# efirdc/Segmentation-Pipeline

Hardware: AMD Instinct MI355X
Metric: 3D patches/sec (128³, 4ch) train+infer at 1/2/4/8 MI355X; Dice vs CPU ref (higher is better)
Workload: dtype f32 (tensors, results and accumulation; the products of the 3x3x3 convolutions with >= 8 input channels run as six bf16 MFMAs on an EXACT three-way bf16 split of both f32 operands -- error vs f64 equal to the f32 MFMA kernels', profiles/r04_f32x3_accuracy.txt; the same step on v_mfma_f32_32x32x2_f32

## Files before the change

### include/m355seg.h

```cpp
#ifndef M355SEG_H
#define M355SEG_H

#include <stddef.h>
#include <stdint.h>

#ifdef __cplusplus
extern "C" {
#endif

#define M355_ABI_VERSION 3

enum {
  M355_OK = 0,
  M355_EINVALID_ARG = -1,
  M355_EUNSUPPORTED = -2,
  M355_ELAUNCH = -3,
  M355_EWORKSPACE = -4
};

enum { M355_F32 = 0 };

enum { M355_COMPUTE_F32 = 0, M355_COMPUTE_BF16 = 1, M355_COMPUTE_F16 = 2, M355_COMPUTE_F32X3 = 3 };

enum { M355_ACT_NONE = 0, M355_ACT_RELU = 1, M355_ACT_LEAKY_RELU = 2, M355_ACT_ELU = 3, M355_ACT_GELU = 4,
// ... 81 lines not shown
size_t m355_conv_transpose3d_workspace(const m355_conv3d_desc* d);
int m355_conv_transpose3d_fwd(const m355_conv3d_desc* d, const float* x, const float* w,
                              const float* bias, float* y,
                              void* workspace, size_t workspace_bytes, void* stream);
int m355_conv_transpose3d_bwd_data(const m355_conv3d_desc* d, const float* dy, const float* w,
                                   float* dx, void* workspace, size_t workspace_bytes,
                                   void* stream);
int m355_conv_transpose3d_bwd_weight(const m355_conv3d_desc* d, const float* x, const float* dy,
                                     float* dw, float* dbias,
                                     void* workspace, size_t workspace_bytes, void* stream);

int m355_conv_transpose3d_plan(const m355_conv3d_desc* d, int32_t which, const void* y_side, int32_t* out4);

int m355_conv_transpose3d_fwd_h16(const m355_conv3d_desc* d, const void* x16, int64_t x16_batch_stride,
                                  const float* w, const float* bias, void* y16, int64_t y16_batch_stride,
                                  int32_t compute, void* stream);

typedef struct m355_norm_desc {
  int32_t N, C;
  int64_t S;
  int32_t groups;
  int32_t act;
  float eps;
  float act_slope;
  int64_t x_batch_stride;
  int64_t y_batch_stride;
  int64_t add_batch_stride;
} m355_norm_desc;

int64_t m355_norm_num_stats(const m355_norm_desc* d);
size_t m355_norm_workspace(const m355_norm_desc* d);

int m355_norm_plan(const m355_norm_desc* d, int32_t which, int32_t* out4);

int m355_norm_stats(const m355_norm_desc* d, const float* x, float* mean, float* rstd,
                    float* running_mean, float* running_var, float momentum,
                    void* workspace, size_t workspace_bytes, void* stream);
int m355_norm_stats_from_partials(const m355_norm_desc* d, const float* stat_partials, int64_t slots,
                                  float* mean, float* rstd, float* running_mean, float* running_var,
                                  float momentum, void* workspace, size_t workspace_bytes, void* stream);
int m355_norm_stats_from_running(const m355_norm_desc* d, const float* running_mean,
                                 const float* running_var, float* mean, float* rstd,
                                 void* stream);
int m355_norm_act_fwd(const m355_norm_desc* d, const float* x, const float* mean,
                      const float* rstd, const float* gamma, const float* beta,
                      const float* add, float* y, void* stream);
int m355_norm_act_pool_fwd(const m355_norm_desc* d, const float* x, const float* mean, const float* rstd,
                           const float* gamma, const float* beta, float* y, float* pooled, int64_t pooled_batch_stride,
                           int32_t D, int32_t H, int32_t W, void* stream);
int m355_norm_act_bwd(const m355_norm_desc* d, const float* x, const float* dy,
                      const float* mean, const float* rstd, const float* gamma,
                      const float* beta, float* dx, float* dgamma, float* dbeta,
                      int training, void* workspace, size_t workspace_bytes, void* stream);
int m355_norm_act_bwd_h16(const m355_norm_desc* d, const float* x, const float* dy, const float* mean,
                          const float* rstd, const float* gamma, const float* beta, float* dx, float* dgamma,
                          float* dbeta, int training, void* dx16, int64_t dx16_batch_stride, int32_t compute,
                          void* workspace, size_t workspace_bytes, void* stream);

int m355_norm_sums(const m355_norm_desc* d, const float* x, const float* stat_partials, int64_t slots, double* sums,
                   void* workspace, size_t workspace_bytes, void* stream);
int m355_norm_stats_from_sums(const m355_norm_desc* d, const double* sums, float* mean, float* rstd,
                              float* running_mean, float* running_var, float momentum, void* stream);
int m355_norm_act_bwd_reduce(const m355_norm_desc* d, const float* x, const float* dy, const float* mean,
                             const float* rstd, const float* gamma, const float* beta, float* dgamma, float* dbeta,
                             int training, const double* total_count, float* stat_m, void* workspace,
                             size_t workspace_bytes, void* stream);
int m355_norm_act_bwd_apply(const m355_norm_desc* d, const float* x, const float* dy, const float* mean,
                            const float* rstd, const float* gamma, const float* beta, const float* stat_m, float* dx,
                            void* dx16, int64_t dx16_batch_stride, int32_t compute, void* stream);

int m355_norm_act_fwd_h16(const m355_norm_desc* d, const float* x, const float* mean, const float* rstd,
                          const float* gamma, const float* beta, const float* add, float* y, void* y16,
                          int64_t y16_batch_stride, int32_t compute, void* stream);
int m355_norm_act_fwd_c8(const m355_norm_desc* d, const void* x16, int64_t x16_batch_stride, const float* mean,
                         const float* rstd, const float* gamma, const float* beta, const void* add16,
                         int64_t add16_batch_stride, void* y16, int64_t y16_batch_stride, int32_t compute,
                         void* stream);
int64_t m355_act16_partials_slots(int64_t S);
int m355_act16_channel_partials(const void* x16, int64_t x16_batch_stride, int32_t N, int32_t C, int64_t S,
                                int32_t compute, float* stat_partials, void* stream);
int m355_avgpool3d_2x_fwd_h16(const void* x16, void* y16, int32_t N, int32_t C, int32_t D, int32_t H, int32_t W,
                              int64_t x16_batch_stride, int64_t y16_batch_stride, int32_t compute, void* stream);

int m355_act16_pack_scaled(const float* x, void* x16, int32_t N, int32_t C, int64_t S, int64_t x_batch_stride,
                           int64_t x16_batch_stride, int32_t compute, float scale, void* stream);
int m355_act16_unpack_scaled(const void* x16, float* x, int32_t N, int32_t C, int64_t S, int64_t x16_batch_stride,
                             int64_t x_batch_stride, int32_t compute, float scale, void* stream);
int m355_conv3d_bwd_data_h16_c8(const m355_conv3d_desc* d, const void* dy16, int64_t dy16_batch_stride, const float* w,
                                void* dx16, int64_t dx16_batch_stride, void* workspace, size_t workspace_bytes,
                                void* stream);
size_t m355_conv3d_bwd_weight_c8_workspace(const m355_conv3d_desc* d);
int m355_conv3d_bwd_weight_c8(const m355_conv3d_desc* d, const void* x16, int64_t x16_batch_stride, const void* dy16,
                              int64_t dy16_batch_stride, float* dw, float* dbias, float grad_unscale, void* workspace,
                              size_t workspace_bytes, void* stream);
int m355_norm_act_bwd_c8(const m355_norm_desc* d, const void* x16, int64_t x16_batch_stride, const void* dy16,
                         int64_t dy16_batch_stride, const void* dpool16, int64_t dpool16_batch_stride, int32_t D,
                         int32_t H, int32_t W, const float* mean, const float* rstd, const float* gamma,
                         const float* beta, void* dx16, int64_t dx16_batch_stride, float* dgamma, float* dbeta,
                         int training, float grad_unscale, int32_t compute, void* workspace, size_t workspace_bytes,
                         void* stream);
int m355_norm_act_bwd_c8_reduce(const m355_norm_desc* d, const void* x16, int64_t x16_batch_stride, const void* dy16,
                                int64_t dy16_batch_stride, const void* dpool16, int64_t dpool16_batch_stride, int32_t D,
                                int32_t H, int32_t W, const float* mean, const float* rstd, const float* gamma,
                                const float* beta, float* dgamma, float* dbeta, int training, const double* total_count,
                                float grad_unscale, float* stat_m, int32_t compute, void* workspace, size_t workspace_bytes,
                                void* stream);
// ... 338 lines not shown
```

### segmentation-pipeline_amd/_lib.py

```python
import ctypes as C
import os

_HERE = os.path.dirname(os.path.abspath(__file__))
LIB_PATH = os.environ.get("M355_LIB_PATH") or os.path.join(_HERE, "libm355seg.so")

M355_OK = 0
ACT_NONE, ACT_RELU, ACT_LEAKY_RELU = 0, 1, 2
ACT_ELU, ACT_GELU, ACT_GELU_TANH, ACT_SILU = 3, 4, 5, 6
COMPUTE_F32, COMPUTE_BF16, COMPUTE_F16, COMPUTE_F32X3 = 0, 1, 2, 3
CONV_W_PACKED, CONV_SOFTMAX, CONV_SIGMOID = 1, 2, 4


class ConvDesc(C.Structure):
    _fields_ = [
        ("N", C.c_int32), ("Cin", C.c_int32), ("Cout", C.c_int32),
        ("D", C.c_int32), ("H", C.c_int32), ("W", C.c_int32),
        ("k", C.c_int32), ("stride", C.c_int32), ("pad", C.c_int32), ("out_pad", C.c_int32),
        ("x_batch_stride", C.c_int64), ("y_batch_stride", C.c_int64),
        ("compute", C.c_int32), ("flags", C.c_int32),
    ]


class PackItem(C.Structure):
    _fields_ = [("desc", ConvDesc), ("which", C.c_int32), ("w", C.c_void_p), ("packed", C.c_void_p)]
# ... 112 lines not shown
    "m355_conv3d_fwd_h16": (C.c_int, [_CD, _P, _i64, _P, _P, _P, _P, _P, _P, _sz, _P]),
    "m355_conv3d_stats_slots_c8": (_i64, [_CD]),
    "m355_conv3d_fwd_h16_c8": (C.c_int, [_CD, _P, _i64, _P, _P, _P, _i64, _P, _P, _sz, _P]),
    "m355_conv3d_bwd_data_h16": (C.c_int, [_CD, _P, _i64, _P, _P, _P, _sz, _P]),
    "m355_conv3d_bwd_weight_h16_workspace": (_sz, [_CD]),
    "m355_conv3d_bwd_weight_h16": (C.c_int, [_CD, _P, _i64, _P, _i64, _P, _P, _P, _P, _sz, _P]),
    "m355_norm_act_fwd_h16": (C.c_int, [_ND, _P, _P, _P, _P, _P, _P, _P, _P, _i64, _i32, _P]),
    "m355_norm_act_fwd_c8": (C.c_int, [_ND, _P, _i64, _P, _P, _P, _P, _P, _i64, _P, _i64, _i32, _P]),
    "m355_act16_partials_slots": (_i64, [_i64]),
    "m355_act16_channel_partials": (C.c_int, [_P, _i64, _i32, _i32, _i64, _i32, _P, _P]),
    "m355_avgpool3d_2x_fwd_h16": (C.c_int, [_P, _P, _i32, _i32, _i32, _i32, _i32, _i64, _i64, _i32, _P]),
    "m355_act16_pack_scaled": (C.c_int, [_P, _P, _i32, _i32, _i64, _i64, _i64, _i32, _f32, _P]),
    "m355_act16_unpack_scaled": (C.c_int, [_P, _P, _i32, _i32, _i64, _i64, _i64, _i32, _f32, _P]),
    "m355_conv3d_bwd_data_h16_c8": (C.c_int, [_CD, _P, _i64, _P, _P, _i64, _P, _sz, _P]),
    "m355_conv3d_bwd_weight_c8_workspace": (_sz, [_CD]),
    "m355_conv3d_bwd_weight_c8": (C.c_int, [_CD, _P, _i64, _P, _i64, _P, _P, _f32, _P, _sz, _P]),
    "m355_norm_act_bwd_c8": (C.c_int, [_ND, _P, _i64, _P, _i64, _P, _i64, _i32, _i32, _i32, _P, _P, _P, _P, _P, _i64, _P, _P,
                                       C.c_int, _f32, _i32, _P, _sz, _P]),
    "m355_norm_act_bwd_c8_reduce": (C.c_int, [_ND, _P, _i64, _P, _i64, _P, _i64, _i32, _i32, _i32, _P, _P, _P, _P, _P, _P,
                                              C.c_int, _P, _f32, _P, _i32, _P, _sz, _P]),
    "m355_norm_act_bwd_c8_apply": (C.c_int, [_ND, _P, _i64, _P, _i64, _P, _i64, _i32, _i32, _i32, _P, _P, _P, _P, _P, _P, _i64,
                                             _i32, _P]),
    "m355_avgpool3d_2x_bwd_h16": (C.c_int, [_P, _P, _P, _i32, _i32, _i32, _i32, _i32, _i64, _i64, _i64, _i32, _P]),
    "m355_upsample_trilinear2x_fwd_h16": (C.c_int, [_P, _P, _i32, _i32, _i32, _i32, _i32, _i64, _i64, _i32, _P]),
    "m355_upsample_trilinear2x_bwd_h16": (C.c_int, [_P, _P, _i32, _i32, _i32, _i32, _i32, _i64, _i64, _i32, _P]),
    "m355_act16_channel_scale": (C.c_int, [_P, _P, _P, _i32, _i32, _i64, _i64, _i64, _i32, _P]),
    "m355_space_to_depth2_h16": (C.c_int, [_P, _P, _i32, _i32, _i32, _i32, _i32, _i64, _i64, _i32, _P]),
    "m355_depth_to_space2_h16": (C.c_int, [_P, _P, _i32, _i32, _i32, _i32, _i32, _i64, _i64, _i32, _P]),
    "m355_conv_transpose3d_h16_bwd_supported": (_i32, [_CD]),
    "m355_conv_transpose3d_h16_bwd_workspace": (_sz, [_CD]),
    "m355_conv_transpose3d_bwd_data_h16": (C.c_int, [_CD, _P, _i64, _P, _P, _i64, _i32, _P]),
    "m355_conv_transpose3d_bwd_weight_h16": (C.c_int, [_CD, _P, _i64, _P, _i64, _P, _P, _f32, _i32, _P, _sz, _P]),
    "m355_conv3d_plan": (C.c_int, [_CD, _i32, C.POINTER(C.c_int32)]),
    "m355_conv3d_launch_plan": (C.c_int, [_i32, _CD, C.POINTER(_i64), C.POINTER(C.c_uint64), _sz, C.POINTER(_i64)]),
    "m355_conv3d_bwd_data_workspace": (_sz, [_CD]),
    "m355_conv3d_bwd_data": (C.c_int, [_CD, _P, _P, _P, _P, _sz, _P]),
    "m355_conv3d_bwd_weight_workspace": (_sz, [_CD]),
    "m355_conv3d_bwd_weight": (C.c_int, [_CD, _P, _P, _P, _P, _P, _sz, _P]),
    "m355_conv_transpose3d_workspace": (_sz, [_CD]),
    "m355_conv_transpose3d_plan": (C.c_int, [_CD, _i32, _P, C.POINTER(C.c_int32)]),
    "m355_conv_transpose3d_fwd": (C.c_int, [_CD, _P, _P, _P, _P, _P, _sz, _P]),
    "m355_conv_transpose3d_bwd_data": (C.c_int, [_CD, _P, _P, _P, _P, _sz, _P]),
    "m355_conv_transpose3d_bwd_weight": (C.c_int, [_CD, _P, _P, _P, _P, _P, _sz, _P]),
    "m355_conv_transpose3d_fwd_h16": (C.c_int, [_CD, _P, _i64, _P, _P, _P, _i64, _i32, _P]),
    "m355_norm_num_stats": (_i64, [_ND]),
    "m355_norm_workspace": (_sz, [_ND]),
    "m355_norm_plan": (C.c_int, [_ND, _i32, C.POINTER(C.c_int32)]),
    "m355_norm_stats": (C.c_int, [_ND, _P, _P, _P, _P, _P, _f32, _P, _sz, _P]),
    "m355_norm_stats_from_partials": (C.c_int, [_ND, _P, _i64, _P, _P, _P, _P, _f32, _P, _sz, _P]),
    "m355_norm_stats_from_running": (C.c_int, [_ND, _P, _P, _P, _P, _P]),
    "m355_norm_act_fwd": (C.c_int, [_ND, _P, _P, _P, _P, _P, _P, _P, _P]),
    "m355_norm_act_pool_fwd": (C.c_int, [_ND, _P, _P, _P, _P, _P, _P, _P, _i64, _i32, _i32, _i32, _P]),
    "m355_norm_act_bwd": (C.c_int, [_ND, _P, _P, _P, _P, _P, _P, _P, _P, _P, C.c_int, _P, _sz, _P]),
    "m355_norm_sums": (C.c_int, [_ND, _P, _P, _i64, _P, _P, _sz, _P]),
    "m355_norm_stats_from_sums": (C.c_int, [_ND, _P, _P, _P, _P, _P, _f32, _P]),
    "m355_norm_act_bwd_reduce": (C.c_int, [_ND, _P, _P, _P, _P, _P, _P, _P, _P, C.c_int, _P, _P, _P, _sz, _P]),
    "m355_norm_act_bwd_apply": (C.c_int, [_ND, _P, _P, _P, _P, _P, _P, _P, _P, _P, _i64, _i32, _P]),
    "m355_norm_act_bwd_h16": (C.c_int, [_ND, _P, _P, _P, _P, _P, _P, _P, _P, _P, C.c_int, _P, _i64, _i32, _P, _sz, _P]),
    "m355_resample_plan": (C.c_int, [_i32, _i32, _i32, _i32, _i32, _i32, C.POINTER(_i64), C.POINTER(C.c_uint64), _i32,
                                     C.POINTER(_i64)]),
    "m355_avgpool3d_2x_fwd": (C.c_int, [_P, _P, _i32, _i32, _i32, _i32, _i32, _i64, _i64, _P]),
    "m355_avgpool3d_2x_bwd": (C.c_int, [_P, _P, _i32, _i32, _i32, _i32, _i32, _i64, _i64, _P]),
    "m355_avgpool3d_2x_bwd_add": (C.c_int, [_P, _P, _P, _i32, _i32, _i32, _i32, _i32, _i64, _i64, _i64, _P]),
    "m355_maxpool3d_2x_fwd": (C.c_int, [_P, _P, _P, _i32, _i32, _i32, _i32, _i32, _i64, _i64, _P]),
    "m355_maxpool3d_2x_bwd": (C.c_int, [_P, _P, _P, _P, _i32, _i32, _i32, _i32, _i32, _i64, _i64, _i64, _P]),
    "m355_maxpool3d_2x_fwd_h16": (C.c_int, [_P, _P, _P, _i32, _i32, _i32, _i32, _i32, _i64, _i64, _i32, _P]),
    "m355_maxpool3d_2x_bwd_h16": (C.c_int, [_P, _P, _P, _P, _i32, _i32, _i32, _i32, _i32, _i64, _i64, _i64, _i32, _P]),
    "m355_upsample_trilinear2x_fwd": (C.c_int, [_P, _P, _i32, _i32, _i32, _i32, _i32, _i64, _i64, _P]),
    "m355_upsample_trilinear2x_bwd": (C.c_int, [_P, _P, _i32, _i32, _i32, _i32, _i32, _i64, _i64, _P]),
    "m355_upsample_nearest2x_fwd": (C.c_int, [_P, _P, _i32, _i32, _i32, _i32, _i32, _i64, _i64, _P]),
    "m355_upsample_nearest2x_bwd": (C.c_int, [_P, _P, _i32, _i32, _i32, _i32, _i32, _i64, _i64, _P]),
    "m355_upsample_trilinear2x_hp_fwd": (C.c_int, [_P, _P, _i32, _i32, _i32, _i32, _i32, _i64, _i64, _P]),
    "m355_upsample_trilinear2x_hp_bwd": (C.c_int, [_P, _P, _i32, _i32, _i32, _i32, _i32, _i64, _i64, _P]),
    "m355_upsample_nearest2x_fwd_h16": (C.c_int, [_P, _P, _i32, _i32, _i32, _i32, _i32, _i64, _i64, _i32, _P]),
    "m355_upsample_nearest2x_bwd_h16": (C.c_int, [_P, _P, _i32, _i32, _i32, _i32, _i32, _i64, _i64, _i32, _P]),
    "m355_upsample_trilinear2x_hp_fwd_h16": (C.c_int, [_P, _P, _i32, _i32, _i32, _i32, _i32, _i64, _i64, _i32, _P]),
    "m355_upsample_trilinear2x_hp_bwd_h16": (C.c_int, [_P, _P, _i32, _i32, _i32, _i32, _i32, _i64, _i64, _i32, _P]),
    "m355_upsample2x_plan": (C.c_int, [_i32, _i32, _i32, _i32, _i32, _i32, _i32, _i32, C.POINTER(_i64), C.POINTER(C.c_uint64),
                                       _i32, C.POINTER(_i64)]),
    "m355_softmax_fwd": (C.c_int, [_P, _P, _i32, _i32, _i32, _i64, _f32, _P]),
    "m355_softmax_bwd": (C.c_int, [_P, _P, _P, _i32, _i32, _i32, _i64, _P]),
    "m355_sigmoid_fwd": (C.c_int, [_P, _P, _i64, _P]),
    "m355_sigmoid_bwd": (C.c_int, [_P, _P, _P, _i64, _P]),
    "m355_hybrid_loss_workspace": (_sz, [_i32, _i32, _i64]),
    "m355_hybrid_loss_fwd": (C.c_int, [_P, _P, _i32, _i32, _i64, _f32, _P, _i32, _P, _P, _P, _sz, _P]),
    "m355_hybrid_loss_bwd": (C.c_int, [_P, _P, _P, _P, _i32, _i32, _i64, _f32, _P, _i32, _P, _P]),
    "m355_binary_loss_workspace": (_sz, [_i32, _i32, _i64]),
    "m355_binary_loss_fwd": (C.c_int, [_P, _P, _i32, _i32, _i64, _f32, _P, _P, _i32, _i32, _P, _P, _P, _sz, _P]),
    "m355_binary_loss_bwd": (C.c_int, [_P, _P, _P, _P, _i32, _i32, _i64, _f32, _P, _P, _i32, _i32, _P, _P]),
    "m355_copy_channels": (C.c_int, [_P, _P, _i32, _i32, _i64, _i64, _i64, _P]),
    "m355_channel_scale": (C.c_int, [_P, _P, _P, _i32, _i32, _i64, _P]),
    "m355_add": (C.c_int, [_P, _P, _P, _i64, _P]),
    "m355_space_to_depth2": (C.c_int, [_P, _P, _i32, _i32, _i32, _i32, _i32, _i64, _i64, _P]),
    "m355_depth_to_space2": (C.c_int, [_P, _P, _i32, _i32, _i32, _i32, _i32, _i64, _i64, _P]),
    "m355_blur_weight_fwd": (C.c_int, [_P, _P, _P, _P, _i32, _i32, _i32, _i32, _P]),
    "m355_blur_weight_bwd": (C.c_int, [_P, _P, _P, _P, _P, _i32, _i32, _i32, _i32, _P]),
    "m355_weight_standardize_fwd": (C.c_int, [_P, _P, _P, _i32, _i32, _P]),
    "m355_weight_standardize_bwd": (C.c_int, [_P, _P, _P, _P, _i32, _i32, _P]),
    "m355_sampler_table_bytes": (_sz, [_i32, _i32, _i32]),
    "m355_sampler_build": (C.c_int, [_P] + [_i32] * 6 + [_P, _P]),
    "m355_sampler_draw": (C.c_int, [_P, _P] + [_i32] * 6 + [_P, _i32, _P, _P]),
    "m355_patch_gather": (C.c_int, [_P, _P, _P] + [_i32] * 8 + [_P]),
    "m355_patch_aggregate_grid": (C.c_int, [_P, _P, _i32, _i32, _i32, _P] + [_i32] * 10 + [_P]),
    "m355_patch_aggregate_grid_weighted": (C.c_int, [_P, _P, _i32, _i32, _i32, _P, _P] + [_i32] * 10 + [_P]),
    "m355_patch_accumulate": (C.c_int, [_P, _P, _P, _P] + [_i32] * 8 + [_P]),
    "m355_patch_gather_padded": (C.c_int, [_P, _P, _P] + [_i32] * 12 + [_f32, _P]),
# ... 148 lines not shown
```

### segmentation-pipeline_amd/csrc/norm.hip

```cpp
#include "norm_host.hpp"
#include "activation.hpp"

namespace m355 {

__device__ __forceinline__ int64_t stat_base(int64_t s, int64_t run, int groups, int C, int64_t S,
                                             int64_t xbs, int64_t len) {
  if (groups == 0) return run * xbs + s * S;
  const int64_t n = s / groups, g = s % groups;
  return n * xbs + g * len;
}

template <bool VEC>
__global__ __launch_bounds__(256) void norm_partial_kernel(const float* __restrict__ x,
                                                           double* __restrict__ partial,
                                                           int groups, int C, int64_t S,
                                                           int64_t xbs, int64_t runs, int64_t len,
                                                           int nblk) {
  __shared__ double scratch[4];
  const int64_t s = blockIdx.y;
  const int b = blockIdx.x;
  const int64_t count = runs * len;
  const int64_t begin = (int64_t)b * NORM_CHUNK;
  const int64_t end = min(count, begin + NORM_CHUNK);
  constexpr int STEP = VEC ? 4 : 1;
// ... 301 lines not shown
    const int64_t items = (int64_t)N * nblk;
    for (int64_t i = lane; i < items; i += 64) {
      const int64_t n = i / nblk, k = i - n * nblk;
      a += partial[((n * C + c) * nblk + k) * 2];
      bb += partial[((n * C + c) * nblk + k) * 2 + 1];
    }
    a = wave_sum(a);
    bb = wave_sum(bb);
    if (lane == 0) {
      if (dbeta) dbeta[c] = (float)(a * (double)grad_unscale);
      if (dgamma) dgamma[c] = (float)(bb * (double)grad_unscale);
      report_nonfinite((float)(a * (double)grad_unscale), oflag);
      report_nonfinite((float)(bb * (double)grad_unscale), oflag);
    }
  }
}

template <bool VEC, bool SMOOTH>
__global__ __launch_bounds__(256) void norm_bwd_apply_kernel(
    const float* __restrict__ x, const float* __restrict__ dy, const float* __restrict__ mean,
    const float* __restrict__ rstd, const float* __restrict__ gamma, const float* __restrict__ beta,
    const float* __restrict__ stat_m, float* __restrict__ dx, int C, int64_t S, int groups, int act,
    float slope, int64_t xbs, int64_t ybs) {
  const int c = blockIdx.y, n = blockIdx.z;
  const int64_t s = groups == 0 ? c : (int64_t)n * groups + c / (C / groups);
  const float m = mean[s], r = rstd[s];
  const float g = gamma ? gamma[c] : 1.f, bt = beta ? beta[c] : 0.f;
  const float m1 = stat_m[s * 2], m2 = stat_m[s * 2 + 1];
  const float* xp = x + (int64_t)n * xbs + (int64_t)c * S;
  const float* dp = dy + (int64_t)n * ybs + (int64_t)c * S;
  float* op = dx + (int64_t)n * xbs + (int64_t)c * S;
  const float sc = r * g, sh = bt - m * sc;
  auto f = [&](float xv, float dv) {
    const float xh = (xv - m) * r;
    const float pre = fmaf(xv, sc, sh);
    const float gg = dv * act_grad<SMOOTH>(pre, act, slope) * g;
    return r * (gg - m1 - xh * m2);
  };
  if (VEC) {
    const int64_t S4 = S >> 2;
    for (int64_t i = blockIdx.x * 256ll + threadIdx.x; i < S4; i += gridDim.x * 256ll) {
      const float4 xv = reinterpret_cast<const float4*>(xp)[i];
      const float4 dv = reinterpret_cast<const float4*>(dp)[i];
      float4 o;
      o.x = f(xv.x, dv.x); o.y = f(xv.y, dv.y); o.z = f(xv.z, dv.z); o.w = f(xv.w, dv.w);
      reinterpret_cast<float4*>(op)[i] = o;
    }
  } else {
    for (int64_t i = blockIdx.x * 256ll + threadIdx.x; i < S; i += gridDim.x * 256ll)
      op[i] = f(xp[i], dp[i]);
  }
}


static void launch_partial(const m355_norm_desc* d, const NormPlan& p, const float* x, double* partial, hipStream_t st) {
  const NormLaunch L = norm_pass(d, p, NORM_STATS, (uintptr_t)x);
  with_bool(L.vec, [&](auto V) {
    hipLaunchKernelGGL(norm_partial_kernel<decltype(V)::value>, L.grid, dim3(256), 0, st, x, partial, d->groups, d->C, d->S,
                       p.xbs, p.runs, p.len, L.nblk);
  });
}

static int64_t partials_items(const m355_norm_desc* d, int64_t slots) {
  return (d->groups == 0 ? (int64_t)d->N : 1) * slots * (d->groups == 0 ? 1 : d->C / d->groups);
}
static int launch_from_partials(const m355_norm_desc* d, const NormPlan& p, const float* part, int64_t slots, double* partial,
                                hipStream_t st) {
  const int nblk = (int)std::max<int64_t>(1, std::min<int64_t>(p.nblk, ceil_div(partials_items(d, slots), 2048)));
  hipLaunchKernelGGL(norm_from_partials_kernel, dim3((unsigned)nblk, (unsigned)p.nstats), dim3(256), 0, st, part, partial,
                     d->groups, d->N, d->C, slots, nblk);
  return nblk;
}

static void launch_finalize(const m355_norm_desc* d, const NormPlan& p, const double* partial, int nblk, float* mean,
                            float* rstd, float* running_mean, float* running_var, float momentum, const double* count_ptr,
                            hipStream_t st) {
  hipLaunchKernelGGL(norm_finalize_kernel, dim3((unsigned)p.nstats), dim3(64), 0, st, partial, mean, rstd, running_mean,
                     running_var, momentum, d->eps, p.nstats, nblk, p.count, count_ptr);
}

static int check_stats(const m355_norm_desc* d, const NormPlan& p, const char* who, size_t workspace_bytes, bool running) {
  M355_REQUIRE(workspace_bytes >= p.workspace_bytes, M355_EWORKSPACE, "%s: workspace too small", who);
  M355_REQUIRE(d->groups == 0 || !running, M355_EINVALID_ARG, "%s: running statistics are only defined for batch norm", who);
  M355_REQUIRE(p.nstats <= 65535, M355_EUNSUPPORTED, "%s: too many statistics", who);
  return M355_OK;
}

int launch_norm_bwd_reduce(const m355_norm_desc* d, const NormPlan& p, const double* partial, const float* gamma, float* dgamma,
                           float* dbeta, float* stat_m, int training, const double* count_ptr, float grad_unscale, int* oflag,
                           hipStream_t st) {
  hipLaunchKernelGGL(norm_bwd_reduce_kernel, dim3((unsigned)std::max<int64_t>(p.nstats, d->C)), dim3(64), 0, st, partial,
                     gamma, dgamma, dbeta, stat_m, d->N, d->C, d->groups, p.bwd().nblk, p.count, training, count_ptr,
                     grad_unscale, oflag);
  return check_launch("norm_bwd_reduce");
}

static int bwd_reduce_half(const m355_norm_desc* d, const NormPlan& p, const float* x, const float* dy, const float* mean,
                           const float* rstd, const float* gamma, const float* beta, float* dgamma, float* dbeta, int training,
                           const double* count_ptr, float* stat_m, void* workspace, size_t workspace_bytes, hipStream_t st,
                           const char* who) {
  M355_REQUIRE(x && dy && mean && rstd && workspace && stat_m, M355_EINVALID_ARG, "%s: null pointer", who);
  M355_REQUIRE(workspace_bytes >= p.workspace_bytes, M355_EWORKSPACE, "%s: workspace too small", who);
  const NormLaunch L = norm_pass(d, p, NORM_BWD1, (uintptr_t)x | (uintptr_t)dy);
  with_bool(L.vec, [&](auto V) {
    with_bool(act_is_smooth(d->act), [&](auto SM) {
      hipLaunchKernelGGL((norm_bwd_partial_kernel<decltype(V)::value, decltype(SM)::value>), L.grid, dim3(256), 0, st, x, dy, mean,
                         rstd, gamma, beta, p.partial(workspace), d->C, d->S, d->groups, d->act, d->act_slope, p.xbs, p.ybs,
                         L.nblk);
    });
  });
  return launch_norm_bwd_reduce(d, p, p.partial(workspace), gamma, dgamma, dbeta, stat_m, training, count_ptr, 1.f, nullptr, st);
}

static int bwd_apply_half(const m355_norm_desc* d, const NormPlan& p, const float* x, const float* dy, const float* mean,
                          const float* rstd, const float* gamma, const float* beta, const float* stat_m, float* dx, void* dx16,
                          int64_t dx16_batch_stride, int compute, hipStream_t st, const char* who) {
  M355_REQUIRE(x && dy && mean && rstd && dx && stat_m, M355_EINVALID_ARG, "%s: null pointer", who);
  if (dx16)
    return launch_norm_bwd_apply_c8(d, p, x, dy, mean, rstd, gamma, beta, stat_m, dx, dx16, p.bs16(dx16_batch_stride), compute,
                                    st);
  const NormLaunch L = norm_pass(d, p, NORM_BWD2, (uintptr_t)x | (uintptr_t)dy | (uintptr_t)dx);
  with_bool(L.vec, [&](auto V) {
    with_bool(act_is_smooth(d->act), [&](auto SM) {
      hipLaunchKernelGGL((norm_bwd_apply_kernel<decltype(V)::value, decltype(SM)::value>), L.grid, dim3(256), 0, st, x, dy, mean,
                         rstd, gamma, beta, stat_m, dx, d->C, d->S, d->groups, d->act, d->act_slope, p.xbs, p.ybs);
    });
  });
  return check_launch(who);
}

static bool dx16_ok(const void* dx16, int64_t dx16_batch_stride, int32_t compute) {
  return (compute == M355_COMPUTE_BF16 || compute == M355_COMPUTE_F16) && ((uintptr_t)dx16 & 15) == 0 &&
         dx16_batch_stride % 8 == 0;
}

static int norm_act_bwd_impl(const m355_norm_desc* d, const float* x, const float* dy, const float* mean, const float* rstd,
                             const float* gamma, const float* beta, float* dx, float* dgamma, float* dbeta, int training,
                             void* workspace, size_t workspace_bytes, void* stream, void* dx16, int64_t dx16_batch_stride,
                             int compute) {
  M355_REQUIRE(d && workspace && dx, M355_EINVALID_ARG, "norm_act_bwd: null pointer");
  if (int rc = validate_norm(d, "norm_act_bwd", NORM_F32)) return rc;
  const NormPlan p = plan_norm(d, dx16 ? NORM_F32_C8 : NORM_F32);
  float* stat_m = p.stat_m(workspace);
  if (int rc = bwd_reduce_half(d, p, x, dy, mean, rstd, gamma, beta, dgamma, dbeta, training, nullptr, stat_m, workspace,
                               workspace_bytes, (hipStream_t)stream, "norm_act_bwd"))
    return rc;
  return bwd_apply_half(d, p, x, dy, mean, rstd, gamma, beta, stat_m, dx, dx16, dx16_batch_stride, compute,
                        (hipStream_t)stream, "norm_act_bwd");
}

}

using namespace m355;

extern "C" int64_t m355_norm_num_stats(const m355_norm_desc* d) {
  if (!d) return 0;
  return d->groups == 0 ? d->C : (int64_t)d->N * d->groups;
}

extern "C" size_t m355_norm_workspace(const m355_norm_desc* d) {
  if (!d || d->N <= 0 || d->C <= 0 || d->S <= 0) return 0;
  return plan_norm(d, NORM_F32).workspace_bytes;
}

extern "C" int m355_norm_plan(const m355_norm_desc* d, int32_t which, int32_t* out4) {
  M355_REQUIRE(d && out4, M355_EINVALID_ARG, "norm_plan: null pointer");
  M355_REQUIRE(which >= 0 && which < NORM_PASS_COUNT, M355_EINVALID_ARG, "norm_plan: no pass %d", which);
  const NormPass pass = (NormPass)which;
  const NormLayout layout = (pass == NORM_FWD_C8 || pass >= NORM_BWD1_C8) ? NORM_C8 : pass == NORM_FWD_H16 ? NORM_F32_C8 : NORM_F32;
  if (int rc = validate_norm(d, "norm_plan", layout)) return rc;
  const NormPlan p = plan_norm(d, layout);
  const NormLaunch L = norm_pass(d, p, pass);
  out4[0] = L.vec;
  out4[1] = L.nblk;
  out4[2] = (int32_t)L.grid.x;
  out4[3] = pass < NORM_BWD1 ? 0 : (int32_t)std::min<size_t>(p.bwd().stat_m_off, INT32_MAX);
  return M355_OK;
}

extern "C" int m355_norm_stats(const m355_norm_desc* d, const float* x, float* mean, float* rstd,
                               float* running_mean, float* running_var, float momentum,
                               void* workspace, size_t workspace_bytes, void* stream) {
  if (int rc = validate_norm(d, "norm_stats", NORM_F32)) return rc;
  M355_REQUIRE(x && mean && rstd && workspace, M355_EINVALID_ARG, "norm_stats: null pointer");
  const NormPlan p = plan_norm(d, NORM_F32);
  if (int rc = check_stats(d, p, "norm_stats", workspace_bytes, running_mean || running_var)) return rc;
  hipStream_t st = (hipStream_t)stream;
  launch_partial(d, p, x, p.partial(workspace), st);
  launch_finalize(d, p, p.partial(workspace), p.nblk, mean, rstd, running_mean, running_var, momentum, nullptr, st);
  return check_launch("norm_stats");
}

extern "C" int m355_norm_stats_from_partials(const m355_norm_desc* d, const float* stat_partials, int64_t slots,
                                             float* mean, float* rstd, float* running_mean,
                                             float* running_var, float momentum, void* workspace,
                                             size_t workspace_bytes, void* stream) {
  if (int rc = validate_norm(d, "norm_stats_from_partials", NORM_F32)) return rc;
  M355_REQUIRE(stat_partials && mean && rstd && workspace && slots > 0, M355_EINVALID_ARG,
               "norm_stats_from_partials: null pointer / no slots");
  const NormPlan p = plan_norm(d, NORM_F32);
  if (int rc = check_stats(d, p, "norm_stats_from_partials", workspace_bytes, running_mean || running_var)) return rc;
  hipStream_t st = (hipStream_t)stream;
  if (partials_items(d, slots) <= 8192) {
    hipLaunchKernelGGL(norm_from_partials_final_kernel, dim3((unsigned)p.nstats), dim3(1024), 0, st, stat_partials, mean,
                       rstd, running_mean, running_var, momentum, d->eps, d->groups, d->N, d->C, slots, p.count);
    return check_launch("norm_stats_from_partials");
// ... 124 lines not shown
```

### segmentation-pipeline_amd/ops.py

```python
import ctypes as C
import os
import weakref
from dataclasses import dataclass
from typing import List, Optional, Sequence

import numpy as np
import torch

from . import _lib
from ._lib import ACT_LEAKY_RELU, ACT_NONE, ACT_RELU, ConvDesc, NormDesc, check

FP32_SPLIT = os.environ.get("M355_FP32_SPLIT", "1") != "0"
_COMPUTE = {"fp32": _lib.COMPUTE_F32X3 if FP32_SPLIT else _lib.COMPUTE_F32, "fp32_mfma": _lib.COMPUTE_F32,
            "bf16": _lib.COMPUTE_BF16, "fp16": _lib.COMPUTE_F16}
_DT16 = {_lib.COMPUTE_BF16: torch.bfloat16, _lib.COMPUTE_F16: torch.float16}
_compute_mode = "fp32"


def set_precision(mode: str):
    global _compute_mode
    if mode not in _COMPUTE:
        raise ValueError(f"precision must be one of {sorted(_COMPUTE)}, not {mode!r}")
    _compute_mode = mode

# ... 349 lines not shown


_deferred = {}


def _adapt_after_overflow(hit: int):
    global _fp16_target, _fp16_clean_checks
    if hit:
        _fp16_calibration.clear()
        _fp16_target = max(_fp16_target / 4.0, 2.0 ** -6)
        _fp16_clean_checks = 0
    else:
        _fp16_clean_checks += 1
        if _fp16_clean_checks >= 200 and _fp16_target < _FP16_TARGET_MAX:
            _fp16_target = min(_FP16_TARGET_MAX, _fp16_target * 2.0)
            _fp16_calibration.clear()
            _fp16_clean_checks = 0


def fp16_found_inf(device) -> Optional[torch.Tensor]:
    idx = device.index if device.index is not None else torch.cuda.current_device()
    w = _overflow_words.get(idx)
    if w is None:
        return None
    d = _deferred.get(idx)
    if d is None:
        d = _deferred[idx] = _DeferredOverflow()
        d.host = torch.zeros(1, dtype=torch.int32).pin_memory()
        d.event = torch.cuda.Event()
    elif d.armed and d.event.query():
        _adapt_after_overflow(int(d.host[0]))
        d.armed = False
    found = (w != 0).to(torch.float32).reshape(())
    if not d.armed:
        d.host.copy_(w, non_blocking=True)
        d.event.record()
        d.armed = True
    w.zero_()
    return found


def fp16_overflow(device=None) -> int:
    hit = 0
    for idx, w in _overflow_words.items():
        if device is not None and device.index not in (None, idx):
            continue
        v = int(w.item())
        if v:
            w.zero_()
            hit |= v
    _adapt_after_overflow(hit)
    return hit
FUSE_POOL = os.environ.get("M355_FUSE_POOL", "1") != "0"


_pack_registry = {}
PACK_BATCH = os.environ.get("M355_PACK_BATCH", "1") != "0"
_pack_scope = None


class pack_scope:
    def __init__(self, params):
        self.ids = {id(p) for p in params}
        self.params = list(params)

    def __enter__(self):
        global _pack_scope
        self.prev, _pack_scope = _pack_scope, self.ids
        for p in self.params:
            cache = getattr(p, "_m355_packed", None)
            if cache is not None:
                p._m355_packed = (-1, cache[1], cache[2])
        return self

    def __exit__(self, *exc):
        global _pack_scope
        _pack_scope = self.prev


def _repack_stale(L, device):
    items = []
    for key, ref in list(_pack_registry.items()):
        if _pack_scope is not None and key not in _pack_scope:
            continue
        w = ref()
        cache = getattr(w, "_m355_packed", None) if w is not None else None
        if cache is None or cache[1] != w.data_ptr() or w.device != device:
            if w is None or cache is None or cache[1] != w.data_ptr():
                del _pack_registry[key]
            continue
        if cache[0] == w._version:
            continue
        for (which, *_), (buf, d) in cache[2].items():
            items.append(_lib.PackItem(d, which, w.data_ptr(), buf.data_ptr()))
        w._m355_packed = (w._version, cache[1], cache[2])
    if items:
        arr = (_lib.PackItem * len(items))(*items)
        check(L.m355_conv3d_pack_batch(C.cast(arr, C.c_void_p), len(items), _stream()), "conv3d_pack_batch")


def _packed_weight(weight, d, which):
    if not PACK_CACHE:
        return weight, 0
    L = _lib.lib()
    ver, ptr = weight._version, weight.data_ptr()
    cache = getattr(weight, "_m355_packed", None)
# ... 1009 lines not shown
    def backward(ctx, dy):
        L = _lib.lib()
        x, mean, rstd, gamma, beta = ctx.saved_tensors
        d0 = ctx.desc
        dy, dybs = _dense_channels(dy)
        d = NormDesc(d0.N, d0.C, d0.S, d0.groups, d0.act, d0.eps, d0.act_slope, d0.x_batch_stride, dybs, 0)
        dx = torch.empty_like(x)
        dgamma = torch.empty(d0.C, dtype=torch.float32, device=x.device) if ctx.has_affine else None
        dbeta = torch.empty(d0.C, dtype=torch.float32, device=x.device) if ctx.has_affine else None
        if ctx.dx_twin:
            dx16 = Act16.empty(d0.N, d0.C, tuple(x.shape[2:]), ctx.dx_twin, x.device)
            _norm_backward(L, d, x, dy, mean, rstd, gamma, beta, dx, dgamma, dbeta, ctx.batch_stats, ctx.sync, dx16,
                           ctx.dx_twin)
            dx._m355_c8 = (dx16, dx._version)
        else:
            _norm_backward(L, d, x, dy, mean, rstd, gamma, beta, dx, dgamma, dbeta, ctx.batch_stats, ctx.sync)
        dadd = dy if (ctx.has_add and ctx.needs_input_grad[3]) else None
        return dx, dgamma, dbeta, dadd, None


class _NormActPoolFn(torch.autograd.Function):

    @staticmethod
    def forward(ctx, x, gamma, beta, cfg: NormCfg):
        L = _lib.lib()
        _require(x, gamma, beta)
        x, xbs = _dense_channels(x)
        N, Cc, D, H, W = x.shape
        S = D * H * W
        if xbs != Cc * S:
            x, xbs = x.contiguous(), Cc * S
        x, xbs = _pairs_in(x, xbs)
        y = _alloc_out(cfg.out, x.shape, x)
        y, ybs = _dense_channels(y)
        yw, ywbs = _pairs_out(y, ybs)
        pooled = torch.empty((N, Cc, D // 2, H // 2, W // 2), dtype=x.dtype, device=x.device)
        d = NormDesc(N, Cc, S, cfg.groups, cfg.act, cfg.eps, cfg.slope, xbs, ywbs, 0)
        mean, rstd, use_batch = _norm_statistics(L, d, x, cfg, N, Cc)
        check(L.m355_norm_act_pool_fwd(C.byref(d), _p(x), _p(mean), _p(rstd), _p(gamma), _p(beta), _p(yw), _p(pooled), 0,
                                       D, H, W, _stream()), "norm_act_pool_fwd")
        if yw is not y:
            y.copy_(yw)
        ctx.desc, ctx.batch_stats, ctx.has_affine, ctx.dims = d, use_batch, gamma is not None, (D, H, W)
        ctx.sync = cfg.sync
        ctx.save_for_backward(x, mean, rstd, gamma, beta)
        return y, pooled

    @staticmethod
    def backward(ctx, dy, dpool):
        L = _lib.lib()
        x, mean, rstd, gamma, beta = ctx.saved_tensors
        d0 = ctx.desc
        D, H, W = ctx.dims
        if dpool is not None:
            dpool, gpbs = _dense_channels(dpool)
            tot = torch.empty_like(x)
            if dy is None:
                check(L.m355_avgpool3d_2x_bwd(_p(dpool), _p(tot), d0.N, d0.C, D, H, W, gpbs, 0, _stream()), "avgpool3d_2x_bwd")
            else:
                dy, gsbs = _dense_channels(dy)
                check(L.m355_avgpool3d_2x_bwd_add(_p(dpool), _p(dy), _p(tot), d0.N, d0.C, D, H, W, gpbs, gsbs, 0,
                                                  _stream()), "avgpool3d_2x_bwd_add")
            dy = tot
        dy, dybs = _dense_channels(dy)
        d = NormDesc(d0.N, d0.C, d0.S, d0.groups, d0.act, d0.eps, d0.act_slope, d0.x_batch_stride, dybs, 0)
        dx = torch.empty_like(x)
        dgamma = torch.empty(d0.C, dtype=torch.float32, device=x.device) if ctx.has_affine else None
        dbeta = torch.empty(d0.C, dtype=torch.float32, device=x.device) if ctx.has_affine else None
        _norm_backward(L, d, x, dy, mean, rstd, gamma, beta, dx, dgamma, dbeta, ctx.batch_stats, ctx.sync)
        return dx, dgamma, dbeta, None


def norm_act_pool(x, gamma, beta, cfg: NormCfg):
    return _NormActPoolFn.apply(x, gamma, beta, cfg)


def norm_act(x, gamma, beta, cfg: NormCfg, add=None, pool=False):
    if cfg.c8 and torch.is_grad_enabled():
        if not isinstance(x, Act16):
            x = pack_act16(x, cfg.c8)
        return _norm_act_c8_train(x, gamma, beta, add, cfg, pool=pool)
    if pool:
        raise _lib.M355Error("norm_act(pool=True) is the c8 training flow's fused pool; use norm_act_pool for fp32 tensors")
    if cfg.c8 and not torch.is_grad_enabled():
        return _norm_act_c8(x, gamma, beta, add, cfg)
    x = as_f32(x)
    cfg.dx_twin = getattr(x, "_m355_c8_grad", 0) if torch.is_grad_enabled() else 0
    y = _NormActFn.apply(x, gamma, beta, as_f32(add) if add is not None else None, cfg)
    if cfg.twin is not None:
        y._m355_c8 = (cfg.twin, y._version)
        cfg.twin = None
    return y


class _AvgPoolFn(torch.autograd.Function):
    @staticmethod
    def forward(ctx, x, out):
        L = _lib.lib()
        _require(x)
        x, xbs = _dense_channels(x)
        N, Cc, D, H, W = x.shape
        y = _alloc_out(out, (N, Cc, D // 2, H // 2, W // 2), x)
        y, ybs = _dense_channels(y)
        check(L.m355_avgpool3d_2x_fwd(_p(x), _p(y), N, Cc, D, H, W, xbs, ybs, _stream()), "avgpool3d_2x_fwd")
        ctx.shape = (N, Cc, D, H, W)
        return y
# ... 1179 lines not shown
```

Before: 50.01.

## Fuse avg-pool backward into norm-activation backward kernels

```diff
diff --git a/include/m355seg.h b/include/m355seg.h
--- a/include/m355seg.h
+++ b/include/m355seg.h
@@ -157,6 +157,11 @@
                       const float* mean, const float* rstd, const float* gamma,
                       const float* beta, float* dx, float* dgamma, float* dbeta,
                       int training, void* workspace, size_t workspace_bytes, void* stream);
+int m355_norm_act_bwd_pool(const m355_norm_desc* d, const float* x, const float* dskip, int64_t dskip_batch_stride,
+                           const float* dpool, int64_t dpool_batch_stride, int32_t D, int32_t H, int32_t W,
+                           const float* mean, const float* rstd, const float* gamma, const float* beta, float* dx,
+                           float* dgamma, float* dbeta, int training, void* workspace, size_t workspace_bytes,
+                           void* stream);
 int m355_norm_act_bwd_h16(const m355_norm_desc* d, const float* x, const float* dy, const float* mean,
                           const float* rstd, const float* gamma, const float* beta, float* dx, float* dgamma,
                           float* dbeta, int training, void* dx16, int64_t dx16_batch_stride, int32_t compute,
diff --git a/segmentation-pipeline_amd/_lib.py b/segmentation-pipeline_amd/_lib.py
--- a/segmentation-pipeline_amd/_lib.py
+++ b/segmentation-pipeline_amd/_lib.py
@@ -188,6 +188,8 @@
     "m355_norm_act_fwd": (C.c_int, [_ND, _P, _P, _P, _P, _P, _P, _P, _P]),
     "m355_norm_act_pool_fwd": (C.c_int, [_ND, _P, _P, _P, _P, _P, _P, _P, _i64, _i32, _i32, _i32, _P]),
     "m355_norm_act_bwd": (C.c_int, [_ND, _P, _P, _P, _P, _P, _P, _P, _P, _P, C.c_int, _P, _sz, _P]),
+    "m355_norm_act_bwd_pool": (C.c_int, [_ND, _P, _P, _i64, _P, _i64, _i32, _i32, _i32, _P, _P, _P, _P, _P, _P, _P, C.c_int,
+                                         _P, _sz, _P]),
     "m355_norm_sums": (C.c_int, [_ND, _P, _P, _i64, _P, _P, _sz, _P]),
     "m355_norm_stats_from_sums": (C.c_int, [_ND, _P, _P, _P, _P, _P, _f32, _P]),
     "m355_norm_act_bwd_reduce": (C.c_int, [_ND, _P, _P, _P, _P, _P, _P, _P, _P, C.c_int, _P, _P, _P, _sz, _P]),
diff --git a/segmentation-pipeline_amd/csrc/norm.hip b/segmentation-pipeline_amd/csrc/norm.hip
--- a/segmentation-pipeline_amd/csrc/norm.hip
+++ b/segmentation-pipeline_amd/csrc/norm.hip
@@ -377,6 +377,121 @@
   }
 }
 
+struct PoolGradSrc {
+  const float* ds;
+  const float* dp;
+  uint32_t W, HW, OW, OHW;
+  __device__ __forceinline__ uint32_t pooled(uint32_t i) const {
+    const uint32_t z = i / HW, rem = i - z * HW;
+    const uint32_t y = rem / W, xw = rem - y * W;
+    return (z >> 1) * OHW + (y >> 1) * OW + (xw >> 1);
+  }
+  __device__ __forceinline__ float one(uint32_t i) const {
+    const float g = dp[pooled(i)] * 0.125f;
+    return ds ? ds[i] + g : g;
+  }
+  template <bool GVEC>
+  __device__ __forceinline__ float4 four(uint32_t i) const {
+    if (GVEC) {
+      const uint32_t q = pooled(i);
+      const float g0 = dp[q] * 0.125f, g1 = dp[q + 1] * 0.125f;
+      if (!ds) return make_float4(g0, g0, g1, g1);
+      const float4 a = *reinterpret_cast<const float4*>(ds + i);
+      return make_float4(a.x + g0, a.y + g0, a.z + g1, a.w + g1);
+    }
+    return make_float4(one(i), one(i + 1), one(i + 2), one(i + 3));
+  }
+};
+
+__device__ __forceinline__ PoolGradSrc pool_grad_src(const float* dskip, int64_t dsbs, const float* dpool, int64_t dpbs,
+                                                     int n, int c, int64_t S, int H, int W) {
+  PoolGradSrc g;
+  g.ds = dskip ? dskip + (int64_t)n * dsbs + (int64_t)c * S : nullptr;
+  g.dp = dpool + (int64_t)n * dpbs + (int64_t)c * (S >> 3);
+  g.W = (uint32_t)W;
+  g.HW = (uint32_t)H * (uint32_t)W;
+  g.OW = (uint32_t)W >> 1;
+  g.OHW = ((uint32_t)H >> 1) * g.OW;
+  return g;
+}
+
+template <bool MAP4, bool GVEC, bool SMOOTH>
+__global__ __launch_bounds__(256) void norm_bwd_partial_pool_kernel(
+    const float* __restrict__ x, const float* __restrict__ dskip, const float* __restrict__ dpool,
+    const float* __restrict__ mean, const float* __restrict__ rstd, const float* __restrict__ gamma,
+    const float* __restrict__ beta, double* __restrict__ partial, int C, int64_t S, int H, int W, int groups, int act,
+    float slope, int64_t xbs, int64_t dsbs, int64_t dpbs, int nblk) {
+  __shared__ double scratch[4];
+  const int b = blockIdx.x, c = blockIdx.y, n = blockIdx.z;
+  const int64_t s = groups == 0 ? c : (int64_t)n * groups + c / (C / groups);
+  const float m = mean[s], r = rstd[s];
+  const float g = gamma ? gamma[c] : 1.f, bt = beta ? beta[c] : 0.f;
+  const float* xp = x + (int64_t)n * xbs + (int64_t)c * S;
+  const PoolGradSrc src = pool_grad_src(dskip, dsbs, dpool, dpbs, n, c, S, H, W);
+  const int64_t begin = (int64_t)b * NORM_CHUNK, end = min(S, begin + NORM_CHUNK);
+  float a1 = 0.f, a2 = 0.f;
+  const float sc = r * g, sh = bt - m * sc;
+  auto acc = [&](float xv, float dv) {
+    const float xh = (xv - m) * r;
+    const float pre = fmaf(xv, sc, sh);
+    const float gg = dv * act_grad<SMOOTH>(pre, act, slope);
+    a1 += gg;
+    a2 = fmaf(gg, xh, a2);
+  };
+  if (MAP4) {
+    for (int64_t i = begin + threadIdx.x * 4; i < end; i += 1024) {
+      const float4 xv = *reinterpret_cast<const float4*>(xp + i);
+      const float4 dv = src.four<GVEC>((uint32_t)i);
+      acc(xv.x, dv.x); acc(xv.y, dv.y); acc(xv.z, dv.z); acc(xv.w, dv.w);
+    }
+  } else {
+    for (int64_t i = begin + threadIdx.x; i < end; i += 256) acc(xp[i], src.one((uint32_t)i));
+  }
+  const double t1 = block_sum<double, 256>((double)a1, scratch);
+  const double t2 = block_sum<double, 256>((double)a2, scratch);
+  if (threadIdx.x == 0) {
+    const int64_t o = (((int64_t)n * C + c) * nblk + b) * 2;
+    partial[o] = t1;
+    partial[o + 1] = t2;
+  }
+}
+
+template <bool MAP4, bool GVEC, bool SMOOTH>
+__global__ __launch_bounds__(256) void norm_bwd_apply_pool_kernel(
+    const float* __restrict__ x, const float* __restrict__ dskip, const float* __restrict__ dpool,
+    const float* __restrict__ mean, const float* __restrict__ rstd, const float* __restrict__ gamma,
+    const float* __restrict__ beta, const float* __restrict__ stat_m, float* __restrict__ dx, int C, int64_t S, int H,
+    int W, int groups, int act, float slope, int64_t xbs, int64_t dsbs, int64_t dpbs) {
+  const int c = blockIdx.y, n = blockIdx.z;
+  const int64_t s = groups == 0 ? c : (int64_t)n * groups + c / (C / groups);
+  const float m = mean[s], r = rstd[s];
+  const float g = gamma ? gamma[c] : 1.f, bt = beta ? beta[c] : 0.f;
+  const float m1 = stat_m[s * 2], m2 = stat_m[s * 2 + 1];
+  const float* xp = x + (int64_t)n * xbs + (int64_t)c * S;
+  float* op = dx + (int64_t)n * xbs + (int64_t)c * S;
+  const PoolGradSrc src = pool_grad_src(dskip, dsbs, dpool, dpbs, n, c, S, H, W);
+  const float sc = r * g, sh = bt - m * sc;
+  auto f = [&](float xv, float dv) {
+    const float xh = (xv - m) * r;
+    const float pre = fmaf(xv, sc, sh);
+    const float gg = dv * act_grad<SMOOTH>(pre, act, slope) * g;
+    return r * (gg - m1 - xh * m2);
+  };
+  if (MAP4) {
+    const int64_t S4 = S >> 2;
+    for (int64_t i = blockIdx.x * 256ll + threadIdx.x; i < S4; i += gridDim.x * 256ll) {
+      const float4 xv = reinterpret_cast<const float4*>(xp)[i];
+      const float4 dv = src.four<GVEC>((uint32_t)(i * 4));
+      float4 o;
+      o.x = f(xv.x, dv.x); o.y = f(xv.y, dv.y); o.z = f(xv.z, dv.z); o.w = f(xv.w, dv.w);
+      reinterpret_cast<float4*>(op)[i] = o;
+    }
+  } else {
+    for (int64_t i = blockIdx.x * 256ll + threadIdx.x; i < S; i += gridDim.x * 256ll)
+      op[i] = f(xp[i], src.one((uint32_t)i));
+  }
+}
+
 
 static void launch_partial(const m355_norm_desc* d, const NormPlan& p, const float* x, double* partial, hipStream_t st) {
   const NormLaunch L = norm_pass(d, p, NORM_STATS, (uintptr_t)x);
@@ -474,9 +589,61 @@
                         (hipStream_t)stream, "norm_act_bwd");
 }
 
+static int norm_act_bwd_pool_impl(const m355_norm_desc* d0, const float* x, const float* dskip, int64_t dskip_bs,
+                                  const float* dpool, int64_t dpool_bs, int D, int H, int W, const float* mean,
+                                  const float* rstd, const float* gamma, const float* beta, float* dx, float* dgamma,
+                                  float* dbeta, int training, void* workspace, size_t workspace_bytes, hipStream_t st) {
+  const char* who = "norm_act_bwd_pool";
+  if (int rc = validate_norm(d0, who, NORM_F32)) return rc;
+  M355_REQUIRE(x && dpool && mean && rstd && dx && workspace, M355_EINVALID_ARG, "%s: null pointer", who);
+  M355_REQUIRE(D > 0 && H > 0 && W > 0 && (int64_t)D * H * W == d0->S, M355_EINVALID_ARG, "%s: D*H*W != desc->S", who);
+  M355_REQUIRE(D % 2 == 0 && H % 2 == 0 && W % 2 == 0, M355_EUNSUPPORTED, "%s: odd spatial size (%d,%d,%d)", who, D, H, W);
+  M355_REQUIRE(d0->S <= INT32_MAX, M355_EUNSUPPORTED, "%s: more than 2^31 - 1 voxels per channel", who);
+  m355_norm_desc dd = *d0;
+  dd.y_batch_stride = 0;
+  const m355_norm_desc* d = &dd;
+  const NormPlan p = plan_norm(d, NORM_F32);
+  M355_REQUIRE(workspace_bytes >= p.workspace_bytes, M355_EWORKSPACE, "%s: workspace too small", who);
+  const int64_t dsbs = dense_or(dskip_bs, (int64_t)d->C * d->S), dpbs = dense_or(dpool_bs, (int64_t)d->C * (d->S / 8));
+  const bool gvec = W % 4 == 0 && (!dskip || (((uintptr_t)dskip & 15) == 0 && dsbs % 4 == 0));
+  float* stat_m = p.stat_m(workspace);
+  auto variant = [&](bool map4, auto&& launch) {
+    with_bool(act_is_smooth(d->act), [&](auto SM) {
+      if (map4 && gvec) launch(std::true_type{}, std::true_type{}, SM);
+      else if (map4) launch(std::true_type{}, std::false_type{}, SM);
+      else launch(std::false_type{}, std::false_type{}, SM);
+    });
+  };
+  const NormLaunch L1 = norm_pass(d, p, NORM_BWD1, (uintptr_t)x);
+  variant(L1.vec, [&](auto M4, auto GV, auto SM) {
+    hipLaunchKernelGGL((norm_bwd_partial_pool_kernel<decltype(M4)::value, decltype(GV)::value, decltype(SM)::value>), L1.grid,
+                       dim3(256), 0, st, x, dskip, dpool, mean, rstd, gamma, beta, p.partial(workspace), d->C, d->S, H, W,
+                       d->groups, d->act, d->act_slope, p.xbs, dsbs, dpbs, L1.nblk);
+  });
+  if (int rc = launch_norm_bwd_reduce(d, p, p.partial(workspace), gamma, dgamma, dbeta, stat_m, training, nullptr, 1.f, nullptr,
+                                      st))
+    return rc;
+  const NormLaunch L2 = norm_pass(d, p, NORM_BWD2, (uintptr_t)x | (uintptr_t)dx);
+  variant(L2.vec, [&](auto M4, auto GV, auto SM) {
+    hipLaunchKernelGGL((norm_bwd_apply_pool_kernel<decltype(M4)::value, decltype(GV)::value, decltype(SM)::value>), L2.grid,
+                       dim3(256), 0, st, x, dskip, dpool, mean, rstd, gamma, beta, stat_m, dx, d->C, d->S, H, W, d->groups,
+                       d->act, d->act_slope, p.xbs, dsbs, dpbs);
+  });
+  return check_launch(who);
+}
+
 }
 
 using namespace m355;
+
+extern "C" int m355_norm_act_bwd_pool(const m355_norm_desc* d, const float* x, const float* dskip, int64_t dskip_batch_stride,
+                                      const float* dpool, int64_t dpool_batch_stride, int32_t D, int32_t H, int32_t W,
+                                      const float* mean, const float* rstd, const float* gamma, const float* beta, float* dx,
+                                      float* dgamma, float* dbeta, int training, void* workspace, size_t workspace_bytes,
+                                      void* stream) {
+  return norm_act_bwd_pool_impl(d, x, dskip, dskip_batch_stride, dpool, dpool_batch_stride, D, H, W, mean, rstd, gamma, beta,
+                                dx, dgamma, dbeta, training, workspace, workspace_bytes, (hipStream_t)stream);
+}
 
 extern "C" int64_t m355_norm_num_stats(const m355_norm_desc* d) {
   if (!d) return 0;
diff --git a/segmentation-pipeline_amd/ops.py b/segmentation-pipeline_amd/ops.py
--- a/segmentation-pipeline_amd/ops.py
+++ b/segmentation-pipeline_amd/ops.py
@@ -425,6 +425,8 @@
     _adapt_after_overflow(hit)
     return hit
 FUSE_POOL = os.environ.get("M355_FUSE_POOL", "1") != "0"
+FUSE_POOL_BWD = os.environ.get("M355_FUSE_POOL_BWD", "1") != "0"
+fused_bwd_counts = {"pool": 0}
 
 
 _pack_registry = {}
@@ -1540,6 +1542,20 @@
         x, mean, rstd, gamma, beta = ctx.saved_tensors
         d0 = ctx.desc
         D, H, W = ctx.dims
+        if dpool is not None and FUSE_POOL_BWD and ctx.sync is None:
+            dpool, gpbs = _dense_channels(dpool)
+            gsbs = 0
+            if dy is not None:
+                dy, gsbs = _dense_channels(dy)
+            dx = torch.empty_like(x)
+            dgamma = torch.empty(d0.C, dtype=torch.float32, device=x.device) if ctx.has_affine else None
+            dbeta = torch.empty(d0.C, dtype=torch.float32, device=x.device) if ctx.has_affine else None
+            ws = _workspace(L.m355_norm_workspace(C.byref(d0)), x.device)
+            check(L.m355_norm_act_bwd_pool(C.byref(d0), _p(x), _p(dy), gsbs, _p(dpool), gpbs, D, H, W, _p(mean), _p(rstd),
+                                           _p(gamma), _p(beta), _p(dx), _p(dgamma), _p(dbeta), 1 if ctx.batch_stats else 0,
+                                           _p(ws), ws.numel(), _stream()), "norm_act_bwd_pool")
+            fused_bwd_counts["pool"] += 1
+            return dx, dgamma, dbeta, None
         if dpool is not None:
             dpool, gpbs = _dense_channels(dpool)
             tot = torch.empty_like(x)
```

Result: faster. 50.52, median of 6 (+1.0%).
